# submarine0418/underwater_image_enhancement

Hardware: AMD Instinct MI355X
Metric: megapixels/sec enhanced (higher is better)
Workload: dtype f32/f64

## Files before the change

include/uwie.h:

```cpp
#ifndef UWIE_H_
#define UWIE_H_

#include <stddef.h>
#include <stdint.h>

#ifdef __cplusplus
extern "C" {
#endif

#define UWIE_OK 0
#define UWIE_E_INVALID (-1)
#define UWIE_E_WORKSPACE (-2)
#define UWIE_E_HIP (-3)
#define UWIE_E_NODEVICE (-4)
#define UWIE_E_DEVICE (-5)

#define UWIE_SURFACE_SIX 0
#define UWIE_SURFACE_DICT 1

#define UWIE_DICT_STRONG_DEHAZING 0
#define UWIE_DICT_MEDIUM_DEHAZING 1
#define UWIE_DICT_LIGHT_ENHANCEMENT 2
#define UWIE_DICT_CLAHE_ENHANCEMENT 3
#define UWIE_DICT_HISTOGRAM_EQUALIZATION 4
// ... 211 lines not shown
#define UWIE_MODEL_RF 0
#define UWIE_MODEL_GB 1
#define UWIE_MODEL_SVC 2
typedef struct uwie_model_desc {
    int32_t kind, n_features, n_classes, n_trees, n_nodes, n_sv;
    const double *mean, *scale;
    const int32_t *tree_offset, *left, *right, *feature;
    const double *threshold;
    const uint8_t *missing_left;
    const double *value;
    double learning_rate;
    const double *init;
    const double *sv, *dual_coef, *intercept;
    const int32_t *n_support;
    const double *prob_a, *prob_b;
    double gamma;
} uwie_model_desc;
typedef struct uwie_model uwie_model;

int uwie_model_check(const uwie_model_desc *desc);
int uwie_model_create(uwie_ctx *ctx, const uwie_model_desc *desc, uwie_model **out_model);
void uwie_model_destroy(uwie_model *model);
int uwie_model_info(const uwie_model *model, int *kind, int *n_classes, int *n_features);

int uwie_classify_f64(uwie_ctx *ctx, const uwie_model *model, const double *d_rows, int batch, int n_features, int32_t *d_label,
                      double *d_proba, void *stream);
size_t uwie_workspace_bytes_predict(int batch, int H, int W);
int uwie_predict_strategy_u8(uwie_ctx *ctx, const uwie_model *model, const uint8_t *d_u8, const float *d_f32, int batch, int H,
                             int W, int gray_shift, int32_t *d_label, double *d_proba, double *d_rows, void *d_workspace,
                             size_t workspace_bytes, void *stream);


int uwie_cast_classify(uwie_ctx *ctx, const uint8_t *d_in, int batch, int H, int W, int32_t *d_kind,
                       float *d_mean_rgb, void *d_workspace, size_t workspace_bytes, void *stream);

int uwie_normalise_correct(uwie_ctx *ctx, const uint8_t *d_in, const int32_t *d_kind, float *d_out_f32, int batch,
                           int H, int W, void *stream);

int uwie_atmospheric_light(uwie_ctx *ctx, const uint8_t *d_in, const int32_t *d_kind, int batch, int H, int W,
                           const uwie_params *p, float *d_A, void *d_trace, void *d_workspace,
                           size_t workspace_bytes, void *stream);

int uwie_transmission_init(uwie_ctx *ctx, const uint8_t *d_in, const int32_t *d_kind, const float *d_A, int batch,
                           int H, int W, const uwie_params *p, float *d_t0, uint8_t *d_gray, void *stream);

int uwie_box_filter_f64(uwie_ctx *ctx, const double *d_src, double *d_dst, int batch, int H, int W, int ksize,
                        void *d_workspace, size_t workspace_bytes, void *stream);

int uwie_guided_filter(uwie_ctx *ctx, const uint8_t *d_gray, const float *d_t0, int batch, int H, int W, int ksize,
                       double eps, int exact, double *d_t, void *d_workspace, size_t workspace_bytes, void *stream);

int uwie_guided_plan(int batch, int H, int W, int ksize, int *split_row0, int *split_rows);

int uwie_restore(uwie_ctx *ctx, const uint8_t *d_in, const int32_t *d_kind, const float *d_A, const double *d_t,
                 int batch, int H, int W, float *d_out_f32, void *stream);

int uwie_percentiles_f32(uwie_ctx *ctx, const float *d_img, int batch, int H, int W, const double *q_percent, int nq,
                         float *d_out, void *d_workspace, size_t workspace_bytes, void *stream);

int uwie_percentiles_f64(uwie_ctx *ctx, const double *d_img, int batch, int H, int W, const double *q_percent, int nq,
                         double *d_out, void *d_workspace, size_t workspace_bytes, void *stream);

int uwie_stretch_f32(uwie_ctx *ctx, const float *d_img, float *d_out, int batch, int H, int W, double lo_percent,
                     double hi_percent, void *d_workspace, size_t workspace_bytes, void *stream);

int uwie_gamma_f32(uwie_ctx *ctx, const float *d_img, float *d_out, size_t n, double g, int mode, void *stream);

int uwie_clahe_f32(uwie_ctx *ctx, const float *d_img, float *d_out, int batch, int H, int W, double clip_limit,
                   int tiles_x, int tiles_y, void *d_workspace, size_t workspace_bytes, void *stream);

int uwie_rgb2gray_u8(uwie_ctx *ctx, const uint8_t *d_rgb, uint8_t *d_gray, size_t npixels, int gray_shift,
                     void *stream);
int uwie_rgb2lab_u8(uwie_ctx *ctx, const uint8_t *d_rgb, uint8_t *d_lab, size_t npixels, void *stream);
int uwie_lab2rgb_u8(uwie_ctx *ctx, const uint8_t *d_lab, uint8_t *d_rgb, size_t npixels, void *stream);
int uwie_clahe_u8(uwie_ctx *ctx, const uint8_t *d_plane, uint8_t *d_out, int batch, int H, int W, double clip_limit,
                  int tiles_x, int tiles_y, void *d_workspace, size_t workspace_bytes, void *stream);
int uwie_canny_u8(uwie_ctx *ctx, const uint8_t *d_gray, uint8_t *d_edges, int batch, int H, int W, int low, int high,
                  void *d_workspace, size_t workspace_bytes, void *stream);
int uwie_equalize_hist_u8(uwie_ctx *ctx, const uint8_t *d_plane, uint8_t *d_out, int batch, int H, int W,
                          void *d_workspace, size_t workspace_bytes, void *stream);

#ifdef __cplusplus
}
#endif
#endif
```

profiles/gf_bench.py:

```python
import os
import sys
import time

import numpy as np
import torch

sys.path.insert(0, os.path.dirname(os.path.dirname(os.path.abspath(__file__))))
import underwater_image_enhancement_amd as uw

H, W, B = (int(v) for v in (sys.argv[1:4] if len(sys.argv) >= 4 else (2160, 3840, 16)))
k = int(sys.argv[4]) if len(sys.argv) > 4 else 15
eps = float(sys.argv[5]) if len(sys.argv) > 5 else 0.5
dev = uw.Device(0)
g = torch.Generator(device="cuda").manual_seed(1)
yy = torch.arange(H, device="cuda").view(1, H, 1)
xx = torch.arange(W, device="cuda").view(1, 1, W)
field = 0.5 + 0.25 * torch.sin(xx / 97.0) * torch.cos(yy / 61.0)
gray = (255 * (field + 0.03 * torch.randn((B, H, W), device="cuda", generator=g)).clamp(0, 1)).to(torch.uint8).contiguous()
t0 = (1.0 - 0.5 * (field * 0.9 + 0.05 * torch.rand((B, H, W), device="cuda", generator=g))).clamp(0.1, 1.0).float().contiguous()


def run(sel, exact=False, reps=5, kk=k):
    dev.tune(gf_split=1, gf_bands=0)
    dev.tune(**sel)
    t = dev.guided_filter(gray, t0, kk, eps, exact=exact)
    torch.cuda.synchronize()
    e0, e1 = torch.cuda.Event(enable_timing=True), torch.cuda.Event(enable_timing=True)
    e0.record()
    for _ in range(reps):
        t = dev.guided_filter(gray, t0, kk, eps, exact=exact)
    e1.record()
    torch.cuda.synchronize()
    return t, e0.elapsed_time(e1) / reps


nb = min(B, 2)
refs = {}
for kk in (k, 7):
    ref, ms_ref = run({}, exact=True, reps=1, kk=kk)
    refs[kk] = ref[:nb].clone()
    print(f"{H}x{W} x{B} k={kk} eps={eps}")
    print(f"  exact-order kernels      {ms_ref:8.3f} ms")
for name, env, mode, kk in (("LDS-tiled strip kernel", {}, False, 7), ("pipe, f64 ring in LDS", {"gf_split": 0}, False, k),
                            ("pipe, f64 split ring", {}, False, k), ("pipe, fx32 ring", {}, 2, k)):
    t, ms = run(env, exact=mode, kk=kk)
    err = (t[:nb] - refs[kk]).abs().max().item()
    gbs = B * H * W * 13 / ms / 1e6
    print(f"  {name:24s} k={kk:2d} {ms:8.3f} ms   {gbs:7.1f} GB/s algorithmic   max|t - t_exact| = {err:.3e}")
```

underwater_image_enhancement_amd/_lib.py:

```python
from __future__ import annotations

import ctypes
import os
import subprocess

_HERE = os.path.dirname(os.path.abspath(__file__))
LIB_PATH = os.path.join(_HERE, "lib", "libuwie.so")
CSRC = os.path.join(_HERE, "csrc")

SURFACE_SIX, SURFACE_DICT = 0, 1
STATUS_DIFF_RANK = 16
STATUS_CLASSIFY_NAN = 64
LOSS_IDENTITY, LOSS_VGG, LOSS_GATED = 0, 1, 2
VGG_F32, VGG_F16, VGG_PARAMS = 0, 1, 1735488
PARAM_NET_PARAMS = {True: 8500100, False: 8459652}
MASKS_GIVEN, MASKS_DRAWN = 0, 1
TRAINER_PARAMS, TRAINER_GRADS, TRAINER_EXP_AVG, TRAINER_EXP_AVG_SQ = 0, 1, 2, 3
FLIP_LR, FLIP_UD = 1, 2
RESIZE_MAX_SIDE, RESIZE_MAX_SRC = 4096, 32768
INTER_F64, INTER_FX32, INTER_F32T = 0, 1, 2
DICT_STRATEGIES = {
    "strong_dehazing": 0,
    "medium_dehazing": 1,
    "light_enhancement": 2,
# ... 21 lines not shown
        ("gf_eps", ctypes.c_double),
        ("L_low", ctypes.c_double),
        ("L_high", ctypes.c_double),
        ("wb_percentile", ctypes.c_double),
        ("clip_limit", ctypes.c_double),
        ("tiles_x", ctypes.c_int32),
        ("tiles_y", ctypes.c_int32),
        ("gamma", ctypes.c_double),
        ("apply_gamma", ctypes.c_int32),
        ("gf_exact", ctypes.c_int32),
        ("inter_dtype", ctypes.c_int32),
    ]


class UwieModelDesc(ctypes.Structure):

    _fields_ = [("kind", ctypes.c_int32), ("n_features", ctypes.c_int32), ("n_classes", ctypes.c_int32),
                ("n_trees", ctypes.c_int32), ("n_nodes", ctypes.c_int32), ("n_sv", ctypes.c_int32),
                ("mean", ctypes.c_void_p), ("scale", ctypes.c_void_p),
                ("tree_offset", ctypes.c_void_p), ("left", ctypes.c_void_p), ("right", ctypes.c_void_p),
                ("feature", ctypes.c_void_p), ("threshold", ctypes.c_void_p), ("missing_left", ctypes.c_void_p),
                ("value", ctypes.c_void_p), ("learning_rate", ctypes.c_double), ("init", ctypes.c_void_p),
                ("sv", ctypes.c_void_p), ("dual_coef", ctypes.c_void_p), ("intercept", ctypes.c_void_p),
                ("n_support", ctypes.c_void_p), ("prob_a", ctypes.c_void_p), ("prob_b", ctypes.c_void_p),
                ("gamma", ctypes.c_double)]


_VP, _SZ, _I, _D = ctypes.c_void_p, ctypes.c_size_t, ctypes.c_int, ctypes.c_double
_PP = ctypes.POINTER(UwieParams)
_PM = ctypes.POINTER(UwieModelDesc)
_PI = ctypes.POINTER(_I)
SIGNATURES = {
    "uwie_last_error": [],
    "uwie_version": [],
    "uwie_create": [_I, ctypes.POINTER(_VP)],
    "uwie_destroy": [_VP],
    "uwie_device_status": [_VP, _VP, ctypes.POINTER(ctypes.c_uint32)],
    "uwie_profile_enable": [_VP, _I],
    "uwie_profile_filter": [_VP, ctypes.c_char_p],
    "uwie_profile_collect": [_VP],
    "uwie_profile_row": [_VP, _I, ctypes.POINTER(ctypes.c_char_p), ctypes.POINTER(_D), ctypes.POINTER(_I)],
    "uwie_params_init": [_PP, _I, _I],
    "uwie_set_tuning": [_VP, ctypes.c_char_p, _I],
    "uwie_get_tuning": [_VP, ctypes.c_char_p, ctypes.POINTER(_I)],
    "uwie_workspace_bytes": [_I, _I, _I, _PP],
    "uwie_workspace_bytes_ctx": [_VP, _I, _I, _I, _PP],
    "uwie_workspace_bytes_all": [_I, _I, _I, _VP],
    "uwie_workspace_bytes_float": [_I, _I, _I, _PP, _I],
    "uwie_enhance_f32": [_VP, _VP, _VP, _VP, _VP, _I, _I, _I, _PP, _VP, _SZ, _VP],
    "uwie_enhance_f64": [_VP, _VP, _VP, _VP, _I, _I, _I, _PP, _VP, _SZ, _VP],
    "uwie_cast_classify_f32": [_VP, _VP, _I, _I, _I, _VP, _VP, _VP],
    "uwie_color_correct_f32": [_VP, _VP, _VP, _VP, _I, _I, _I, _VP],
    "uwie_guided_plan": [_I, _I, _I, _I, ctypes.POINTER(ctypes.c_int), ctypes.POINTER(ctypes.c_int)],
    "uwie_enhance_u8": [_VP, _VP, _VP, _VP, _I, _I, _I, _PP, _VP, _SZ, _VP],
    "uwie_enhance_u8_f64": [_VP, _VP, _VP, _VP, _I, _I, _I, _PP, _VP, _SZ, _VP],
    "uwie_enhance_percentiles": [_VP, _VP, _SZ, _I, _I, _I, _PP, _VP, _VP],
    "uwie_enhance_all_u8": [_VP, _VP, _VP, _VP, _I, _I, _I, _VP, _VP, _SZ, _VP],
    "uwie_workspace_bytes_select": [_I, _I, _I, _VP, _I, _I],
    "uwie_select_best_u8": [_VP, _VP, _I, _I, _I, _VP, _I, _VP, _VP, _VP, _VP, _VP, _VP, _SZ, _VP],
    "uwie_diff_enhance_f32": [_VP, _VP, _VP, _I, _I, _I, _I, _VP, _I, _VP, _SZ, _VP],
    "uwie_diff_enhance_save_f32": [_VP, _VP, _VP, _I, _I, _I, _I, _VP, _I, _VP, _VP, _SZ, _VP],
    "uwie_diff_enhance_bwd_workspace_bytes": [_I, _I, _I],
    "uwie_workspace_bytes_diff_u8": [_I, _I, _I],
    "uwie_diff_enhance_u8": [_VP, _VP, _VP, _VP, _I, _I, _I, _VP, _I, _VP, _VP, _SZ, _VP],
    "uwie_diff_enhance_bwd_f32": [_VP, _VP, _VP, _I, _I, _I, _I, _I, _VP, _VP, _VP, _VP, _VP, _SZ, _VP],
    "uwie_diff_gated_f32": [_VP, _VP, _VP, _I, _I, _I, _I, _VP, _I, _VP, _SZ, _VP],
    "uwie_diff_gated_save_f32": [_VP, _VP, _VP, _I, _I, _I, _I, _VP, _I, _VP, _VP, _SZ, _VP],
    "uwie_diff_gated_bwd_workspace_bytes": [_I, _I, _I],
    "uwie_workspace_bytes_diff_gated_u8": [_I],
    "uwie_diff_gated_u8": [_VP, _VP, _VP, _VP, _I, _I, _I, _VP, _I, _VP, _VP, _SZ, _VP],
    "uwie_diff_gated_bwd_f32": [_VP, _VP, _VP, _I, _I, _I, _I, _I, _VP, _VP, _VP, _VP, _VP, _SZ, _VP],
    "uwie_ref_loss_workspace_bytes": [_I, _I, _I],
    "uwie_ref_loss_f32": [_VP, _I, _VP, _VP, _I, _I, _I, _I, _I, _VP, _VP, _VP, _VP, _VP, _SZ, _VP],
    "uwie_ref_loss_bwd_f32": [_VP, _I, _VP, _VP, _I, _I, _I, _I, _I, _VP, _VP, _VP, _VP, _VP, _VP, _VP, _SZ, _VP],
    "uwie_device_status_async": [_VP, _VP, _VP],
    "uwie_vgg_create": [_VP, _VP, _I, ctypes.POINTER(_VP)],
    "uwie_vgg_destroy": [_VP],
    "uwie_perceptual_workspace_bytes": [_I, _I, _I, _I],
    "uwie_perceptual_f32": [_VP, _VP, _VP, _VP, _I, _I, _I, _VP, _VP, _SZ, _VP],
    "uwie_perceptual_bwd_f32": [_VP, _VP, _I, _I, _I, _VP, _VP, _VP, _SZ, _VP],
    "uwie_param_net_create": [_VP, _VP, _I, ctypes.POINTER(_VP)],
    "uwie_param_net_destroy": [_VP],
    "uwie_param_net_workspace_bytes": [_I, _I, _I],
    "uwie_param_net_f32": [_VP, _VP, _VP, _VP, _I, _I, _I, _VP, _VP, _VP, _SZ, _VP],
    "uwie_mlp_create": [_VP, _VP, _I, _I, _I, ctypes.POINTER(_VP)],
    "uwie_mlp_destroy": [_VP],
    "uwie_mlp_workspace_bytes": [_I, _I],
    "uwie_mlp_forward": [_VP, _VP, _VP, _I, _I, _VP, _VP, _SZ, _VP],
    "uwie_mlp_trainer_create": [_VP, _VP, _I, _I, _I, ctypes.POINTER(_VP)],
    "uwie_mlp_trainer_destroy": [_VP],
    "uwie_mlp_train_workspace_bytes": [_I, _I, _I],
    "uwie_mlp_train_forward": [_VP, _VP, _VP, _I, _I, _D, _I, _VP, ctypes.c_uint64, _VP, _VP, _SZ, _VP],
    "uwie_mlp_backward": [_VP, _VP, _VP, _I, _I, _VP, _VP, _SZ, _VP],
    "uwie_mlp_adam_step": [_VP, _VP, _D, _D, _D, _D, _D, _VP, _VP],
    "uwie_mlp_trainer_get": [_VP, _I, _VP],
    "uwie_mlp_trainer_set": [_VP, _I, _VP],
    "uwie_mlp_trainer_step_count": [_VP],
    "uwie_mlp_trainer_set_step_count": [_VP, ctypes.c_longlong],
    "uwie_mlp_trainer_eval": [_VP, _VP, _VP, _I, _I, _VP, _VP, _SZ, _VP],
    "uwie_u8_to_f32": [_VP, _VP, _VP, _SZ, _VP],
    "uwie_extract_features_u8": [_VP, _VP, _VP, _I, _I, _I, _VP, _SZ, _VP],
    "uwie_feature_extractor_count": [_I, _I],
    "uwie_workspace_bytes_feature_extractor": [_I, _I, _I],
    "uwie_feature_extractor_u8": [_VP, _VP, _VP, _I, _I, _I, _I, _VP, _VP, _SZ, _VP],
    "uwie_model_check": [_PM],
    "uwie_model_create": [_VP, _PM, ctypes.POINTER(_VP)],
# ... 85 lines not shown
```

underwater_image_enhancement_amd/csrc/api.hip:

```cpp
#include <cstdarg>
#include <cstdio>
#include <cstring>
#include <type_traits>

#include "common.h"

#include <cstdlib>

namespace uwie {

static thread_local char g_err[512] = "";
static thread_local uwie_ctx *g_ctx = nullptr;
static const Tuning g_default_tuning{};

const Tuning &tune() { return g_ctx ? g_ctx->tune : g_default_tuning; }
uwie_ctx *current_ctx() { return g_ctx; }

void set_error(const char *fmt, ...)
{
    va_list ap;
    va_start(ap, fmt);
    vsnprintf(g_err, sizeof g_err, fmt, ap);
    va_end(ap);
}
// ... 487 lines not shown
#define UWIE_REQUIRE_F(cond, ...)       \
    do {                                \
        if (!(cond)) {                  \
            set_error(__VA_ARGS__);     \
            return UWIE_E_INVALID;      \
        }                               \
    } while (0)

constexpr int kMlpEvalBatch = 1 << 20, kMlpTrainBatch = 65536;
template <class H>
int mlp_rows_check(const char *who, const uwie_ctx *ctx, const H *h, const void *d_features, int features_are_f64, int batch,
                   bool training, const float *d_other, const char *other_name)
{
    UWIE_REQUIRE_F(ctx && h && d_features && d_other, "%s: NULL pointer", who);
    UWIE_REQUIRE_F(h->device == ctx->device, "%s: the %s lives on another device", who,
                   std::is_same<H, uwie_mlp>::value ? "network" : "trainer");
    UWIE_REQUIRE_F(batch >= 1 && batch <= (training ? kMlpTrainBatch : kMlpEvalBatch), "%s: batch out of range (1 .. %s)", who,
                   training ? "65536" : "2^20");
    UWIE_REQUIRE_F(((uintptr_t)d_features & (features_are_f64 ? 7 : 3)) == 0 && ((uintptr_t)d_other & 3) == 0,
                   "%s: d_features and %s must be aligned for their element types", who, other_name);
    return UWIE_OK;
}

bool module_flags_ok(int map, int flags) { return map == UWIE_LOSS_VGG ? (flags & ~3) == 0 : flags == 0; }
int module_flags_check(const char *who, int map, int flags, bool name_module = false)
{
    const bool vgg = map == UWIE_LOSS_VGG;
    UWIE_REQUIRE_F(module_flags_ok(map, flags), "%s: %sflags are %s", who, !name_module ? "" : vgg ? "vgg " : "gated ",
                   vgg ? "UWIE_DIFF_OMEGA | UWIE_DIFF_GAMMA" : "reserved (0)");
    return UWIE_OK;
}

}
}

using namespace uwie;

extern "C" {

const char *uwie_last_error(void) { return g_err; }
const char *uwie_version(void) { return "uwie 0.1 (gfx950)"; }

int uwie_create(int device, uwie_ctx **out_ctx)
{
    UWIE_REQUIRE(out_ctx != nullptr, "out_ctx is NULL");
    *out_ctx = nullptr;
    int count = 0;
    if (hipGetDeviceCount(&count) != hipSuccess || count <= 0) {
        set_error("no HIP device available (libuwie has no CPU path)");
        return UWIE_E_NODEVICE;
    }
    UWIE_REQUIRE(device >= 0 && device < count, "device index out of range");
    UWIE_HIP_CHECK(hipSetDevice(device));
    uwie_ctx *ctx = new uwie_ctx();
    ctx->aux_ready = false;
    ctx->prof = prof_create();
    ctx->device = device;
    tuning_from_env(&ctx->tune);
    LabTables *lab = new LabTables();
    CastTables *cast = new CastTables();
    build_lab_tables(lab);
    build_cast_tables(cast);
    hipError_t e = hipMalloc((void **)&ctx->d_lab, sizeof(LabTables));
    if (e == hipSuccess) e = hipMalloc((void **)&ctx->d_cast, sizeof(CastTables));
    if (e == hipSuccess) e = hipMalloc((void **)&ctx->d_status, 64);
    if (e == hipSuccess) e = hipMemset(ctx->d_status, 0, 64);
    if (e == hipSuccess) e = hipMemcpy(ctx->d_lab, lab, sizeof(LabTables), hipMemcpyHostToDevice);
    if (e == hipSuccess) e = hipMemcpy(ctx->d_cast, cast, sizeof(CastTables), hipMemcpyHostToDevice);
    delete lab;
    delete cast;
    if (e != hipSuccess) {
        set_error("context table upload failed: %s", hipGetErrorString(e));
        uwie_destroy(ctx);
        return UWIE_E_HIP;
    }
    *out_ctx = ctx;
    return UWIE_OK;
}

void uwie_destroy(uwie_ctx *ctx)
{
    if (!ctx) return;
    if (ctx->d_lab) (void)hipFree(ctx->d_lab);
    if (ctx->d_cast) (void)hipFree(ctx->d_cast);
    if (ctx->d_status) (void)hipFree(ctx->d_status);
    if (ctx->aux_ready) {
        for (int i = 0; i < 4; ++i) {
            (void)hipStreamDestroy(ctx->aux[i]);
            (void)hipEventDestroy(ctx->join[i]);
        }
        (void)hipEventDestroy(ctx->fork);
    }
    prof_bind(nullptr);
    prof_destroy(ctx->prof);
    delete ctx;
}

int uwie_device_status(uwie_ctx *ctx, void *stream, uint32_t *bits)
{
    UWIE_REQUIRE(ctx != nullptr, "device_status: NULL context");
    UWIE_SCOPE(ctx);
    uint32_t v = 0;
    hipStream_t st = (hipStream_t)stream;
    UWIE_HIP_CHECK(hipMemcpyAsync(&v, ctx->d_status, sizeof v, hipMemcpyDeviceToHost, st));
    UWIE_HIP_CHECK(hipStreamSynchronize(st));
    if (v) UWIE_HIP_CHECK(hipMemsetAsync(ctx->d_status, 0, sizeof v, st));
    if (bits) *bits = v;
    if (v) {
        set_error("device status 0x%x:%s the results of the calls since the last check are not valid", v,
                  (v & UWIE_STATUS_CANNY_LABEL) ? " Canny hysteresis met a component label that this launch did not write (k_canny.hip);"
// ... 1202 lines not shown

int uwie_transmission_init(uwie_ctx *ctx, const uint8_t *d_in, const int32_t *d_kind, const float *d_A, int batch, int H,
                           int W, const uwie_params *p, float *d_t0, uint8_t *d_gray, void *stream)
{
    UWIE_REQUIRE(ctx && d_in && d_A && p && (d_t0 || d_gray), "transmission_init: NULL pointer");
    UWIE_SCOPE(ctx);
    UWIE_CHECK_SHAPE(batch, H, W);
    const Shape s{batch, H, W};
    hipStream_t st = (hipStream_t)stream;
    const bool six = p->surface == UWIE_SURFACE_SIX;
    if (d_t0) UWIE_TRY(launch_trans_init(d_in, d_kind, d_A, s, (float)p->omega, six ? 1e-6f : 1e-10f, six ? 1 : 0, d_t0, st));
    if (d_gray) UWIE_TRY(launch_quant_gray(d_in, d_kind, d_gray, s, p->gray_shift, st));
    return UWIE_OK;
}

int uwie_box_filter_f64(uwie_ctx *ctx, const double *d_src, double *d_dst, int batch, int H, int W, int ksize,
                        void *d_workspace, size_t workspace_bytes, void *stream)
{
    UWIE_REQUIRE(ctx && d_src && d_dst, "box_filter: NULL pointer");
    UWIE_SCOPE(ctx);
    UWIE_CHECK_SHAPE(batch, H, W);
    UWIE_REQUIRE(ksize >= 1 && ksize <= 1024, "box_filter: ksize out of range");
    const Shape s{batch, H, W};
    UWIE_CHECK_WS(box_ws_bytes(s));
    return launch_box_filter_f64(d_src, d_dst, s, ksize, d_workspace, (hipStream_t)stream);
}

int uwie_guided_filter(uwie_ctx *ctx, const uint8_t *d_gray, const float *d_t0, int batch, int H, int W, int ksize,
                       double eps, int exact, double *d_t, void *d_workspace, size_t workspace_bytes, void *stream)
{
    UWIE_REQUIRE(ctx && d_gray && d_t0 && d_t, "guided_filter: NULL pointer");
    UWIE_SCOPE(ctx);
    UWIE_CHECK_SHAPE(batch, H, W);
    UWIE_REQUIRE(ksize >= 1 && ksize <= 1024, "guided_filter: ksize out of range");
    const Shape s{batch, H, W};
    UWIE_CHECK_WS(guided_ws_bytes(s));
    UWIE_REQUIRE(exact >= 0 && exact <= 2, "guided_filter: mode is 0 (fused float64), 1 (exact order) or 2 (fixed-point ring)");
    GuidedRequest r{ksize, eps, exact == 1};
    r.fx = exact == 2;
    return launch_guided_plan(plan_guided(s, r), s, d_gray, d_t0, d_t, d_workspace, (hipStream_t)stream);
}

int uwie_guided_plan(int batch, int H, int W, int ksize, int *split_row0, int *split_rows)
{
    UWIE_REQUIRE(split_row0 && split_rows, "guided_plan: NULL pointer");
    UWIE_CHECK_SHAPE(batch, H, W);
    const GuidedPlan g = plan_guided(Shape{batch, H, W}, {ksize, 1.0});
    const bool split = g.route == GF_SPLIT;
    *split_row0 = split ? g.iy0 : 0;
    *split_rows = split ? g.rows : 0;
    return UWIE_OK;
}

int uwie_restore(uwie_ctx *ctx, const uint8_t *d_in, const int32_t *d_kind, const float *d_A, const double *d_t,
                 int batch, int H, int W, float *d_out_f32, void *stream)
{
    UWIE_REQUIRE(ctx && d_in && d_A && d_t && d_out_f32, "restore: NULL pointer");
    UWIE_SCOPE(ctx);
    UWIE_CHECK_SHAPE(batch, H, W);
    return launch_restore(d_in, d_kind, d_A, d_t, Shape{batch, H, W}, d_out_f32, (hipStream_t)stream);
}

int uwie_percentiles_f32(uwie_ctx *ctx, const float *d_img, int batch, int H, int W, const double *q_percent, int nq,
                         float *d_out, void *d_workspace, size_t workspace_bytes, void *stream)
{
    UWIE_REQUIRE(ctx && d_img && q_percent && d_out, "percentiles: NULL pointer");
    UWIE_SCOPE(ctx);
    UWIE_CHECK_SHAPE(batch, H, W);
    const Shape s{batch, H, W};
    UWIE_CHECK_WS(select_ws_bytes(s));
    return launch_percentiles(d_img, 0, s, q_percent, nq, d_out, d_workspace, (hipStream_t)stream);
}

int uwie_percentiles_f64(uwie_ctx *ctx, const double *d_img, int batch, int H, int W, const double *q_percent, int nq,
                         double *d_out, void *d_workspace, size_t workspace_bytes, void *stream)
{
    UWIE_REQUIRE(ctx && d_img && q_percent && d_out, "percentiles_f64: NULL pointer");
    UWIE_SCOPE(ctx);
    UWIE_CHECK_SHAPE(batch, H, W);
    const Shape s{batch, H, W};
    UWIE_CHECK_WS(select_ws_bytes(s));
    return launch_percentiles(d_img, 0, s, q_percent, nq, d_out, d_workspace, (hipStream_t)stream);
}

int uwie_enhance_percentiles(uwie_ctx *ctx, const void *d_workspace, size_t workspace_bytes, int batch, int H, int W,
                             const uwie_params *p, double *d_out, void *stream)
{
    UWIE_REQUIRE(ctx && d_workspace && d_out, "enhance_percentiles: NULL context, workspace or output pointer");
    UWIE_SCOPE(ctx);
    UWIE_CHECK_SHAPE(batch, H, W);
    UWIE_TRY(check_params(p));
    UWIE_REQUIRE(dehazes(p), "enhance_percentiles: only the dehazing strategies select percentiles in the workspace");
    const Shape s{batch, H, W};
    const EnhanceLayout L = carve_enhance(const_cast<void *>(d_workspace), workspace_bytes, s, p, !ctx->last_enhance_f64);
    UWIE_CHECK_WS(L.total);
    hipStream_t st = (hipStream_t)stream;
    const bool dict = p->surface == UWIE_SURFACE_DICT;
    const size_t per = (!dict && p->strategy == 3) ? 4 : 2;
    for (int i = 0; i < L.nsplit; ++i) {
        const size_t n = (size_t)L.cnt[i] * 3 * per;
        double *o = d_out + (size_t)L.start[i] * 3 * per;
        if (dict) UWIE_HIP_CHECK(hipMemcpyAsync(o, L.P[i].pct64, n * sizeof(double), hipMemcpyDeviceToDevice, st));
        else UWIE_TRY(launch_widen_f32(L.P[i].pct, o, n, st));
    }
    return UWIE_OK;
}
// ... 98 lines not shown
```

underwater_image_enhancement_amd/csrc/common.h:

```cpp
#pragma once
#include <hip/hip_runtime.h>
#include <stddef.h>
#include <stdint.h>

#include "../../include/uwie.h"

namespace uwie {

void set_error(const char *fmt, ...);
#define UWIE_HIP_CHECK(expr)                                                            \
    do {                                                                                \
        hipError_t _e = (expr);                                                         \
        if (_e != hipSuccess) {                                                         \
            ::uwie::set_error("%s failed: %s (%s:%d)", #expr, hipGetErrorString(_e), __FILE__, __LINE__); \
            return UWIE_E_HIP;                                                          \
        }                                                                               \
    } while (0)
#define UWIE_LAUNCH_CHECK() UWIE_HIP_CHECK(hipGetLastError())
#define UWIE_REQUIRE(cond, msg)                 \
    do {                                        \
        if (!(cond)) {                          \
            ::uwie::set_error("%s", msg);       \
            return UWIE_E_INVALID;              \
        }                                       \
// ... 16 lines not shown
    uint32_t R[kCastBinades][256];
    uint8_t tie[kCastBinades][256];
    uint32_t RT[256][kCastBinades];
    uint2 RT2[128][kCastBinades];
    uint8_t tiebin[256];
};

void build_lab_tables(LabTables *t);
void build_cast_tables(CastTables *t);

struct Profiler;
Profiler *prof_create();
void prof_destroy(Profiler *p);
void prof_enable(Profiler *p, bool on);
void prof_filter(Profiler *p, const char *name);
void prof_bind(Profiler *p);
int prof_collect(Profiler *p);
int prof_row(Profiler *p, int i, const char **name, double *ms, int *calls);
class ProfScope {
public:
    ProfScope(const char *name, hipStream_t st);
    ~ProfScope();
    ProfScope(const ProfScope &) = delete;

private:
    int rec_;
    hipStream_t st_;
};
#define UWIE_PROF_CAT2(a, b) a##b
#define UWIE_PROF_CAT(a, b) UWIE_PROF_CAT2(a, b)
#define UWIE_PROF(name, st) ::uwie::ProfScope UWIE_PROF_CAT(_uwie_prof_, __LINE__)(name, st)
#define UWIE_LAUNCH_AS(row, kernel, grid, block, lds, st, ...)              \
    do {                                                                    \
        UWIE_PROF(row, st);                                                 \
        hipLaunchKernelGGL(kernel, grid, block, lds, st, __VA_ARGS__);      \
    } while (0)
#define UWIE_LAUNCH(kernel, ...) UWIE_LAUNCH_AS(#kernel, kernel, __VA_ARGS__)

}

namespace uwie {
struct Tuning {
    int gf_split = 1;
    int gf_bands = 0;
    int select_generic = 0;
    int restore_store = 0;
    int lin_predict3 = 0;
    int lin_cap = 0;
    int lin_no_predict = 0;
    int q_hist = 1;
    int lin_predict_shift = 0;
    int streams = 1;
    int canny_prepass = 1;
    int gf_fuse = 0;
    int rank_sweep = 1;
    int canny_fault_inject = 0;
    int entry_fuse = 1;
};
const Tuning &tune();
uwie_ctx *current_ctx();
}

struct uwie_ctx {
    int device;
    uwie::Tuning tune;
    bool attr_q_tail = false;
    bool attr_cast_resolve = false;
    int attr_gf_fast = 0;
    int attr_gf_split8 = 0;
    uwie::LabTables *d_lab;
    uwie::CastTables *d_cast;
    uwie::Profiler *prof;
    uint32_t *d_status = nullptr;
    hipStream_t aux[4];
    hipEvent_t fork, join[4];
    bool aux_ready;
    bool last_enhance_f64 = false;
};

namespace uwie {

struct Carver {
    char *base;
    size_t off;
    explicit Carver(void *b) : base(static_cast<char *>(b)), off(0) {}
    template <typename T>
    T *take(size_t count)
    {
        off = (off + 255) & ~size_t(255);
        T *p = base ? reinterpret_cast<T *>(base + off) : nullptr;
        off += count * sizeof(T);
        return p;
    }
    size_t total() const { return (off + 255) & ~size_t(255); }
};

static inline int cdiv(long long a, long long b) { return (int)((a + b - 1) / b); }
static inline int grid_for(size_t n, size_t cap = 8192)
{
    size_t g = (n + 255) / 256;
    if (g > cap) g = cap;
    return g < 1 ? 1 : (int)g;
}

struct Region {
    int32_t img, y0, x0, rows, cols;
};

struct Shape {
    int B, H, W;
    size_t npx() const { return (size_t)H * W; }
};

size_t cast_ws_bytes(Shape s);
struct EntryFuse {
    uint32_t *qpart;
    uint8_t *gray;
    int32_t *guess;
    int gray_shift;
};
int launch_cast_classify(uwie_ctx *ctx, const uint8_t *d_in, Shape s, int32_t *d_kind, float *d_mean, void *ws,
                         hipStream_t st, const EntryFuse *ef = nullptr);
// ... 56 lines not shown
    const double *svT;
    const double *coef;
    const double *rho;
    const double *prob_a, *prob_b;
    const int32_t *sv_start;
};
int classify_model_check(const uwie_model_desc *d);
size_t classify_blob_bytes(const uwie_model_desc *d);
ClsModel classify_pack(const uwie_model_desc *d, void *host_blob, const void *dev_blob);
int launch_classify(const ClsModel &m, const double *d_rows, int B, int32_t *d_label, double *d_proba, uint32_t *d_status,
                    hipStream_t st);

int launch_pick_best(const double *d_scores, int n, Shape s, const uint8_t *d_all, int32_t *d_best, uint8_t *d_out, hipStream_t st);

size_t guided_ws_bytes(Shape s);
size_t box_ws_bytes(Shape s);
int launch_trans_init(const uint8_t *d_in, const int32_t *d_kind, const float *d_A, Shape s, float omega, float norm_eps,
                      int pre_clip, float *d_t0, hipStream_t st);
int launch_box_filter_f64(const double *d_src, double *d_dst, Shape s, int k, void *ws, hipStream_t st);
int launch_guided(const uint8_t *d_gray, const float *d_t0, Shape s, int k, double eps, double *d_t, void *ws,
                  hipStream_t st);
int launch_guided_p64(const uint8_t *d_gray, const double *d_t0, Shape s, int k, double eps, double *d_t, void *ws, hipStream_t st);

enum GuidedRoute {
    GF_EXACT,
    GF_FAST,
    GF_PIPE,
    GF_SPLIT,
    GF_FUSED,
};
struct GuidedRequest {
    int k;
    double eps;
    bool exact = false;
    bool fx = false;
    bool f32_ok = false;
    bool t0_from_frame = false;
    bool t0_f64 = false;
};
struct GuidedPlan {
    GuidedRoute route;
    int k;
    double eps;
    bool t_f32;
    bool ring_fx;
    bool t0_f64;
    bool t0;
    bool planes;
    int TH;
    int iy0, band, nb, rows;
    int pipe_bands;
};
GuidedPlan plan_guided(Shape s, const GuidedRequest &r);
struct FuseT0Args {
    const uint8_t *rgb;
    const int32_t *kind;
    const float *A;
    float omega, norm_eps;
    int pre_clip;
};
int launch_guided_plan(const GuidedPlan &g, Shape s, const uint8_t *d_gray, const void *d_t0, double *d_t, void *ws, hipStream_t st,
                       const FuseT0Args *frame = nullptr);
int guided_fast_th(Shape s, int k);
int launch_guided_fast(const uint8_t *d_gray, const float *d_t0, Shape s, int k, int TH, double eps, double *d_t, hipStream_t st);

constexpr int kMaxPct = 4;
size_t select_ws_bytes(Shape s);
template <typename V>
int launch_percentiles(const V *d_vals, int planar, Shape s, const double *q_percent, int nq, V *d_out, void *ws, hipStream_t st);
int launch_widen_f32(const float *d_in, double *d_out, size_t n, hipStream_t st);

constexpr int kSelGroupStride = 2 * kMaxPct * 2048;
constexpr int kSelOsStride = 2 * kMaxPct;
struct LinState;
struct SelectPlan {
    void *state;
    uint32_t *ghist;
    void *os;
    double t[kMaxPct];
    int nq;
    bool is64;
    LinState *lin;
    void *lists;
    uint32_t *flags;
    uint32_t cap;
    bool predicted;
    uint32_t ranks[2 * kMaxPct];
    template <typename V>
    V *lists_as() const { return static_cast<V *>(lists); }
};
constexpr int kLinBins = 2050;
__host__ __device__ inline uint32_t lin_digit(float x)
{
    if (!(x > 0.0f)) return 0;
    if (x >= 1.0f) return kLinBins - 1;
    const uint32_t d = (uint32_t)(x * 2048.0f);
    return 1 + (d > 2047u ? 2047u : d);
}
__host__ __device__ inline uint32_t lin_digit(double x)
{
    if (!(x > 0.0)) return 0;
    if (x >= 1.0) return kLinBins - 1;
    const uint32_t d = (uint32_t)(x * 2048.0);
    return 1 + (d > 2047u ? 2047u : d);
}
constexpr int kLinLists = 2 * kMaxPct;
// ... 164 lines not shown
```

underwater_image_enhancement_amd/csrc/k_guided_pipe.hip:

```cpp
#include "common.h"
#include "devutil.h"
#include "guided_wave.h"

#include <algorithm>
#include <cmath>
#include <type_traits>
#include <utility>

namespace uwie {

namespace {

#define UWIE_TRY_RC(call)               \
    do {                                \
        const int _rc = (call);         \
        if (_rc != UWIE_OK) return _rc; \
    } while (0)

#ifndef UWIE_GF_MINBAND
#define UWIE_GF_MINBAND 32
#endif
constexpr int kPipeSlots = 128;
struct PipeGeom {
    int H, W, band;
// ... 905 lines not shown
    int gr = i0 - Lb - 2;
    int yo = y_lo;
    auto issue = [&](In &fill) {
        asm volatile("" : "+s"(re), "+s"(gr), "+s"(yo));
        const uint32_t er = (uint32_t)pipe_reflect(re, H), lr = (uint32_t)pipe_reflect(re - RC, H);
        const uint32_t og = (uint32_t)min(max(gr, 0), H - 1);
        load_rows(er * pitch_t, er * pitch_g, lr * pitch_t, lr * pitch_g, og * pitch_g, fill);
        ++re;
        ++gr;
    };
    In buf[NB];
    [&]<int... Q>(std::integer_sequence<int, Q...>) { (issue(buf[Q]), ...); }(std::make_integer_sequence<int, NB - 1>{});
    auto one = [&](auto warm_tag, auto slot_tag, In &fill, const In &use) {
        issue(fill);
        step(warm_tag, slot_tag, use, (uint32_t)yo * pitch_o, yo < H);
        if constexpr (!decltype(warm_tag)::value) ++yo;
        __builtin_amdgcn_sched_barrier(0);
    };
    auto period = [&](auto warm_tag) {
        auto at = [&](auto slot_tag) {
            constexpr int S = decltype(slot_tag)::value;
            one(warm_tag, slot_tag, buf[(S + NB - 1) % NB], buf[S % NB]);
        };
        [&]<int... Q>(std::integer_sequence<int, Q...>) { (at(IC<Q>{}), ...); }(std::make_integer_sequence<int, RC>{});
    };
    period(std::true_type{});
    const int nper = (((int)bid.y == g.nbands - 1 ? g.y_end - y_lo : g.band) + RC - 1) / RC;
    for (int p = 0; p < nper; ++p) period(std::false_type{});
}


template <int K, typename TOut>
__global__ void __launch_bounds__(64) __attribute__((amdgpu_waves_per_eu(2, 2)))
k_guided_split(const uint8_t *__restrict__ gray, const float *__restrict__ t0, TOut *__restrict__ tout, SplitGeom g, PipeConsts cs)
{
    extern __shared__ double2 lds_raw[];
    char *lds = reinterpret_cast<char *>(lds_raw);
    int3 bid = {(int)blockIdx.x, (int)blockIdx.y, (int)blockIdx.z};
    if (g.xcd_fold) {
        const uint32_t gx = gridDim.x, gy = gridDim.y, n = gx * gy * gridDim.z;
        const uint32_t lin = blockIdx.x + gx * (blockIdx.y + gy * blockIdx.z);
        const uint32_t xcd = lin & 7u, idx = lin >> 3, q = n >> 3, r = n & 7u;
        const uint32_t log = (xcd < r ? xcd * (q + 1) : r * (q + 1) + (xcd - r) * q) + idx;
        bid.x = (int)(log % gx);
        bid.y = (int)((log / gx) % gy);
        bid.z = (int)(log / (gx * gy));
    }
    const int x_lo = bid.x * PipeCfg<K>::NV;
    const bool edge = x_lo - 2 * PipeCfg<K>::a < 0 || x_lo - 2 * PipeCfg<K>::a + kPipeSlots > g.W;
    if (edge) split_body<K, true, TOut>(gray, t0, tout, g, cs, lds, bid);
    else split_body<K, false, TOut>(gray, t0, tout, g, cs, lds, bid);
}

template <int K, typename TOut>
__global__ void __launch_bounds__(512) __attribute__((amdgpu_waves_per_eu(2, 2)))
k_guided_split8(const uint8_t *__restrict__ gray, FuseT0Args fz, TOut *__restrict__ tout, SplitGeom g, PipeConsts cs, int nstrips)
{
    extern __shared__ double2 lds_raw[];
    char *lds = reinterpret_cast<char *>(lds_raw);
    constexpr int per_wave = SplitCfg<K>::lds_bytes;
    float *tab = reinterpret_cast<float *>(lds + 8 * per_wave);
    const int wave = __builtin_amdgcn_readfirstlane((int)(threadIdx.x >> 6)), lane = threadIdx.x & 63;
    int grp = (int)blockIdx.x, b = (int)blockIdx.z;
    if (g.xcd_fold) {
        const uint32_t gx = gridDim.x, n = gx * gridDim.z, lin = blockIdx.x + gx * blockIdx.z;
        const uint32_t xcd = lin & 7u, idx = lin >> 3, q = n >> 3, r = n & 7u;
        const uint32_t log = (xcd < r ? xcd * (q + 1) : r * (q + 1) + (xcd - r) * q) + idx;
        grp = (int)(log % gx);
        b = (int)(log / gx);
    }
    {
        const int kd = fz.kind ? fz.kind[b] : 0;
        for (int i = threadIdx.x; i < 768; i += 512) {
            const int c = i >> 8;
            tab[i] = px_val(i & 255, px_atten(kd, c)) / (fz.A[b * 3 + c] + fz.norm_eps);
        }
    }
    __syncthreads();
    const int item = grp * 8 + wave;
    if (item >= nstrips * g.nbands) return;
    const int3 bid = {item % nstrips, item / nstrips, b};
    const int x_lo = bid.x * PipeCfg<K>::NV;
    const bool edge = x_lo - 2 * PipeCfg<K>::a < 0 || x_lo - 2 * PipeCfg<K>::a + kPipeSlots > g.W;
    const float *t0 = reinterpret_cast<const float *>(fz.rgb);
    if (edge) split_body<K, true, TOut, true>(gray, t0, tout, g, cs, lds + wave * per_wave, bid, lane, tab, fz.omega, fz.pre_clip);
    else split_body<K, false, TOut, true>(gray, t0, tout, g, cs, lds + wave * per_wave, bid, lane, tab, fz.omega, fz.pre_clip);
}

template <int K, typename TOut>
int launch_split8(const uint8_t *d_gray, const FuseT0Args &fz, Shape s, const PipeConsts &cs, TOut *d_t, int y0, int band, int nbands,
                  int y_end, hipStream_t st)
{
    using C = PipeCfg<K>;
    constexpr int lds = 8 * SplitCfg<K>::lds_bytes + 768 * 4;
    static_assert(lds <= 160 * 1024, "eight strips and the table have to fit one CU");
#ifndef UWIE_SPLIT8_FOLD
#define UWIE_SPLIT8_FOLD 1
#endif
    SplitGeom g{s.H, s.W, y0, band, y_end, UWIE_SPLIT8_FOLD, nbands};
    const int nstrips = cdiv(s.W, C::NV);
    uwie_ctx *ctx = current_ctx();
    const int bit = std::is_same<TOut, double>::value ? 1 : 2;
    if (ctx && !(ctx->attr_gf_split8 & bit)) {
        UWIE_HIP_CHECK(hipFuncSetAttribute(reinterpret_cast<const void *>(&k_guided_split8<K, TOut>),
                                           hipFuncAttributeMaxDynamicSharedMemorySize, lds));
        ctx->attr_gf_split8 |= bit;
    }
    {
        UWIE_PROF("k_guided_split8", st);
        hipLaunchKernelGGL((k_guided_split8<K, TOut>), dim3(cdiv((long long)nstrips * nbands, 8), 1, s.B), dim3(512), (size_t)lds, st, d_gray,
                           fz, d_t, g, cs, nstrips);
    }
    UWIE_LAUNCH_CHECK();
    return UWIE_OK;
}

template <int K, typename TOut>
int launch_split(const uint8_t *d_gray, const float *d_t0, Shape s, const PipeConsts &cs, TOut *d_t, int y0, int band, int nbands,
                 int y_end, hipStream_t st)
{
    using C = PipeCfg<K>;
    constexpr int lds = SplitCfg<K>::lds_bytes;
#ifndef UWIE_SPLIT_FOLD
#define UWIE_SPLIT_FOLD 1
#endif
    SplitGeom g{s.H, s.W, y0, band, y_end, UWIE_SPLIT_FOLD, nbands};
    const int nstrips = cdiv(s.W, C::NV);
    {
        UWIE_PROF("k_guided_split", st);
        hipLaunchKernelGGL((k_guided_split<K, TOut>), dim3(nstrips, nbands, s.B), dim3(64), (size_t)lds, st, d_gray, d_t0, d_t, g, cs);
    }
    UWIE_LAUNCH_CHECK();
    return UWIE_OK;
}

template <int K, bool FX, typename TOut>
int launch_pipe(const uint8_t *d_gray, const float *d_t0, Shape s, const PipeConsts &cs, TOut *d_t, int nbands, hipStream_t st,
                const int *border = nullptr)
{
    using C = PipeCfg<K>;
    constexpr int lds = C::lds_bytes(FX);
    const int nstrips = cdiv(s.W, C::NV);
    PipeGeom g{};
    g.H = s.H; g.W = s.W;
    g.band = cdiv(s.H, nbands);
    int gy = cdiv(s.H, g.band);
    if (border) {
        g.iy0 = border[0]; g.iy1 = border[1]; g.iband = border[2];
        gy = 2 + border[3];
        g.is0 = border[4]; g.is1 = border[5];
    }
    {
        UWIE_PROF("k_guided_pipe", st);
        hipLaunchKernelGGL((k_guided_pipe<K, FX, TOut>), dim3(nstrips, gy, s.B), dim3(64), (size_t)lds, st, d_gray, d_t0, d_t, g, cs);
    }
    UWIE_LAUNCH_CHECK();
    return UWIE_OK;
}

int pipe_bands(Shape s, int k, bool fx, int forced)
{
    const int lds = k == 10 ? PipeCfg<10>::lds_bytes(fx) : k == 15 ? PipeCfg<15>::lds_bytes(fx) : PipeCfg<20>::lds_bytes(fx);
    const int resident = 256 * std::max(1, std::min(8, (160 * 1024) / lds));
// ... 45 lines not shown
    const double amax = (se <= 0.5 ? 0.45 / (2.0 * se) : 0.225 / (0.25 + eps)) * 1.02;
    const double hb = (0.45 + amax) * 1.02;
    *Sa = (int)std::floor(std::log2(1073741824.0 / amax));
    *Sb = (int)std::floor(std::log2(1073741824.0 / hb));
    return *Sa >= 28 && *Sb >= 28;
}

PipeConsts pipe_consts(const GuidedPlan &g)
{
    const double K2 = (double)g.k * g.k, scale = 1.0 / K2;
    PipeConsts cs{};
    cs.Ek = 255.0 * K2 * K2 * g.eps;
    cs.kaI = scale / 255.0;
    cs.kb = scale;
    cs.b0 = 0.0;
    int Sa, Sb;
    if (g.ring_fx && fx_scales(g.eps, &Sa, &Sb)) {
        const double fa = std::ldexp(1.0, Sa), fb = std::ldexp(1.0, Sb);
        const double b0i = std::nearbyint(0.55 * fb);
        cs.fxa = fa;
        cs.fxb = scale * fb;
        cs.magic_b = kMagic - b0i;
        cs.kaI = scale / 255.0 / fa;
        cs.kb = scale / fb;
        cs.b0 = b0i / fb;
    }
    return cs;
}

template <int K, typename TOut>
int launch_pipe_plan(const GuidedPlan &g, const uint8_t *d_gray, const float *d_t0, Shape s, const PipeConsts &cs, TOut *d_t,
                     hipStream_t st)
{
    if constexpr (std::is_same<TOut, double>::value)
        if (g.ring_fx) return launch_pipe<K, true, double>(d_gray, d_t0, s, cs, d_t, g.pipe_bands, st);
    if (g.route == GF_PIPE) return launch_pipe<K, false, TOut>(d_gray, d_t0, s, cs, d_t, g.pipe_bands, st);
    UWIE_TRY_RC((launch_split<K, TOut>(d_gray, d_t0, s, cs, d_t, g.iy0, g.band, g.nb, g.iy0 + g.rows, st)));
    if (K & 1) return UWIE_OK;
    const int border[6] = {g.iy0, g.iy0 + g.rows, g.band, 0, 0, 0};
    return launch_pipe<K, false, TOut>(d_gray, d_t0, s, cs, d_t, g.pipe_bands, st, border);
}

template <typename TOut>
int launch_wave(const GuidedPlan &g, const uint8_t *d_gray, const float *d_t0, Shape s, TOut *d_t, hipStream_t st)
{
    const PipeConsts cs = pipe_consts(g);
    if (g.k == 10) return launch_pipe_plan<10>(g, d_gray, d_t0, s, cs, d_t, st);
    if (g.k == 15) return launch_pipe_plan<15>(g, d_gray, d_t0, s, cs, d_t, st);
    return launch_pipe_plan<20>(g, d_gray, d_t0, s, cs, d_t, st);
}

}

GuidedPlan plan_guided(Shape s, const GuidedRequest &r)
{
    GuidedPlan g{};
    g.k = r.k;
    g.eps = r.eps;
    g.t0 = true;
    const bool free_order = !r.exact && !r.t0_f64 && r.k >= 1 && r.k <= 1024;
    const bool wave = free_order && (r.k == 10 || r.k == 15 || r.k == 20) && s.W >= 2 * r.k && s.H >= 4 * r.k && s.B <= 65535 &&
                      r.eps > 0.0;
    if (!wave) {
        g.TH = free_order ? guided_fast_th(s, r.k) : 0;
        g.route = g.TH ? GF_FAST : GF_EXACT;
        g.t0_f64 = r.t0_f64;
        g.planes = !g.TH;
        return g;
    }
    const Tuning &tu = tune();
    int Sa, Sb;
    g.ring_fx = r.fx && fx_scales(r.eps, &Sa, &Sb);
    g.t_f32 = r.f32_ok && !g.ring_fx && !(s.W & 1);
    g.pipe_bands = pipe_bands(s, r.k, g.ring_fx, tu.gf_bands);
    g.route = GF_PIPE;
    if (!g.ring_fx && tu.gf_split && split_plan(s, r.k, tu.gf_bands, &g.iy0, &g.band, &g.nb, &g.rows)) {
        g.route = GF_SPLIT;
        if (r.k == 15 && r.t0_from_frame && !r.fx && tu.gf_fuse) {
            g.route = GF_FUSED;
            g.t0 = false;
        }
    }
    return g;
}

int launch_guided_plan(const GuidedPlan &g, Shape s, const uint8_t *d_gray, const void *d_t0, double *d_t, void *ws, hipStream_t st,
                       const FuseT0Args *frame)
{
    const float *t0 = static_cast<const float *>(d_t0);
    switch (g.route) {
    case GF_EXACT:
        UWIE_REQUIRE(ws, "guided filter: the exact-order kernels need the workspace's planes");
        if (g.t0_f64) return launch_guided_p64(d_gray, static_cast<const double *>(d_t0), s, g.k, g.eps, d_t, ws, st);
        return launch_guided(d_gray, t0, s, g.k, g.eps, d_t, ws, st);
    case GF_FAST: return launch_guided_fast(d_gray, t0, s, g.k, g.TH, g.eps, d_t, st);
    case GF_FUSED:
        UWIE_REQUIRE(frame, "guided filter: the fused plan computes t0 from the frame");
        if (g.t_f32) return launch_split8<15, float>(d_gray, *frame, s, pipe_consts(g), reinterpret_cast<float *>(d_t), g.iy0, g.band, g.nb, s.H, st);
        return launch_split8<15, double>(d_gray, *frame, s, pipe_consts(g), d_t, g.iy0, g.band, g.nb, s.H, st);
    default:
        if (g.t_f32) return launch_wave(g, d_gray, t0, s, reinterpret_cast<float *>(d_t), st);
        return launch_wave(g, d_gray, t0, s, d_t, st);
    }
}

}
```

Baseline: 57860.

## Enable fused t0 guided-filter route by default when strips fill the GPU

Changes the default gf_fuse from 0 to 2. In mode 2 the fused split8 kernel, which computes t0 from the frame inside the guided filter, is chosen only when the number of strip work items covers at least one full round of resident wavefronts (8 per compute unit). The split8 kernel also drops from 8 to 4 waves per block, so two blocks can share a CU and tail blocks can be smaller. A query API and a sweep benchmark are added to compare the fused and unfused routes. The aim is to skip the separate t0 pass and its memory traffic on large batches, while keeping the unfused path for small batches where the fused kernel would leave the GPU underfilled.

```diff
diff --git a/include/uwie.h b/include/uwie.h
--- a/include/uwie.h
+++ b/include/uwie.h
@@ -287,6 +287,8 @@
 
 int uwie_guided_plan(int batch, int H, int W, int ksize, int *split_row0, int *split_rows);
 
+int uwie_guided_fill(int batch, int H, int W, int ksize, long long *items);
+
 int uwie_restore(uwie_ctx *ctx, const uint8_t *d_in, const int32_t *d_kind, const float *d_A, const double *d_t,
                  int batch, int H, int W, float *d_out_f32, void *stream);
 
diff --git a/profiles/gf_bench.py b/profiles/gf_bench.py
--- a/profiles/gf_bench.py
+++ b/profiles/gf_bench.py
@@ -7,6 +7,57 @@
 
 sys.path.insert(0, os.path.dirname(os.path.dirname(os.path.abspath(__file__))))
 import underwater_image_enhancement_amd as uw
+
+
+
+def sweep():
+    import ctypes
+
+    from underwater_image_enhancement_amd import _lib
+
+    REPS = 5
+    dev = uw.Device(0)
+    cus = torch.cuda.get_device_properties(0).multi_processor_count
+    p = dev.params(_lib.SURFACE_SIX, 2)
+    print(f"# gf_fuse = 1 against 0, strategy 2, ms per call (min .. max of three alternating rounds of {REPS} calls); {cus} compute units,")
+    print(f"# resident strip-wavefronts {cus * 8}; default: the route gf_fuse = 2 takes")
+    print("# H W B items rounds | fuse=0 ms | fuse=1 ms | median diff ms | default route")
+    jobs = [(2160, 3840, b) for b in (2, 4, 8, 16, 32, 64)] + [(1080, 1920, b) for b in (10, 64, 128)]
+    for H, W, B in jobs:
+        g = torch.Generator(device="cuda").manual_seed(B)
+        frames = torch.randint(0, 256, (B, H, W, 3), generator=g, device="cuda", dtype=torch.uint8)
+        items = ctypes.c_longlong()
+        _lib.check(dev.lib.uwie_guided_fill(B, H, W, 15, ctypes.byref(items)))
+        ms = {0: [], 1: []}
+        for rnd in range(4):
+            for fuse in (0, 1):
+                with dev.tuning(gf_fuse=fuse):
+                    dev.enhance_u8(frames, p)
+                    e0, e1 = torch.cuda.Event(enable_timing=True), torch.cuda.Event(enable_timing=True)
+                    e0.record()
+                    for _ in range(REPS):
+                        dev.enhance_u8(frames, p)
+                    e1.record()
+                    torch.cuda.synchronize()
+                if rnd:
+                    ms[fuse].append(e0.elapsed_time(e1) / REPS)
+        dev.profile(True)
+        dev.profile_rows()
+        dev.enhance_u8(frames, p)
+        rows = dev.profile_rows()
+        dev.profile(False)
+        route = "fused" if "k_guided_split8" in rows else "split" if "k_guided_split" in rows else "pipe"
+        med = sorted(ms[1])[1] - sorted(ms[0])[1]
+        print(f"{H} {W} {B:3d} {items.value:6d} {items.value / (cus * 8):5.2f} | {min(ms[0]):7.3f} .. {max(ms[0]):7.3f} | "
+              f"{min(ms[1]):7.3f} .. {max(ms[1]):7.3f} | {med:+7.3f} | {route}", flush=True)
+        del frames
+        dev._workspace = None
+        torch.cuda.empty_cache()
+
+
+if len(sys.argv) > 1 and sys.argv[1] == "--sweep":
+    sweep()
+    sys.exit(0)
 
 H, W, B = (int(v) for v in (sys.argv[1:4] if len(sys.argv) >= 4 else (2160, 3840, 16)))
 k = int(sys.argv[4]) if len(sys.argv) > 4 else 15
diff --git a/underwater_image_enhancement_amd/_lib.py b/underwater_image_enhancement_amd/_lib.py
--- a/underwater_image_enhancement_amd/_lib.py
+++ b/underwater_image_enhancement_amd/_lib.py
@@ -97,6 +97,7 @@
     "uwie_cast_classify_f32": [_VP, _VP, _I, _I, _I, _VP, _VP, _VP],
     "uwie_color_correct_f32": [_VP, _VP, _VP, _VP, _I, _I, _I, _VP],
     "uwie_guided_plan": [_I, _I, _I, _I, ctypes.POINTER(ctypes.c_int), ctypes.POINTER(ctypes.c_int)],
+    "uwie_guided_fill": [_I, _I, _I, _I, ctypes.POINTER(ctypes.c_longlong)],
     "uwie_enhance_u8": [_VP, _VP, _VP, _VP, _I, _I, _I, _PP, _VP, _SZ, _VP],
     "uwie_enhance_u8_f64": [_VP, _VP, _VP, _VP, _I, _I, _I, _PP, _VP, _SZ, _VP],
     "uwie_enhance_percentiles": [_VP, _VP, _SZ, _I, _I, _I, _PP, _VP, _VP],
diff --git a/underwater_image_enhancement_amd/csrc/api.hip b/underwater_image_enhancement_amd/csrc/api.hip
--- a/underwater_image_enhancement_amd/csrc/api.hip
+++ b/underwater_image_enhancement_amd/csrc/api.hip
@@ -563,10 +563,13 @@
     }
     UWIE_REQUIRE(device >= 0 && device < count, "device index out of range");
     UWIE_HIP_CHECK(hipSetDevice(device));
+    int cus = 0;
+    UWIE_HIP_CHECK(hipDeviceGetAttribute(&cus, hipDeviceAttributeMultiprocessorCount, device));
     uwie_ctx *ctx = new uwie_ctx();
     ctx->aux_ready = false;
     ctx->prof = prof_create();
     ctx->device = device;
+    ctx->cus = cus;
     tuning_from_env(&ctx->tune);
     LabTables *lab = new LabTables();
     CastTables *cast = new CastTables();
@@ -1875,6 +1878,16 @@
     return UWIE_OK;
 }
 
+int uwie_guided_fill(int batch, int H, int W, int ksize, long long *items)
+{
+    UWIE_REQUIRE(items, "guided_fill: NULL pointer");
+    UWIE_CHECK_SHAPE(batch, H, W);
+    const Shape s{batch, H, W};
+    const GuidedPlan g = plan_guided(s, {ksize, 1.0});
+    *items = g.route == GF_SPLIT ? guided_items(s, g) : 0;
+    return UWIE_OK;
+}
+
 int uwie_restore(uwie_ctx *ctx, const uint8_t *d_in, const int32_t *d_kind, const float *d_A, const double *d_t,
                  int batch, int H, int W, float *d_out_f32, void *stream)
 {
diff --git a/underwater_image_enhancement_amd/csrc/common.h b/underwater_image_enhancement_amd/csrc/common.h
--- a/underwater_image_enhancement_amd/csrc/common.h
+++ b/underwater_image_enhancement_amd/csrc/common.h
@@ -92,7 +92,7 @@
     int lin_predict_shift = 0;
     int streams = 1;
     int canny_prepass = 1;
-    int gf_fuse = 0;
+    int gf_fuse = 2;
     int rank_sweep = 1;
     int canny_fault_inject = 0;
     int entry_fuse = 1;
@@ -108,6 +108,7 @@
     bool attr_cast_resolve = false;
     int attr_gf_fast = 0;
     int attr_gf_split8 = 0;
+    int cus = 0;
     uwie::LabTables *d_lab;
     uwie::CastTables *d_cast;
     uwie::Profiler *prof;
@@ -270,6 +271,7 @@
     int pipe_bands;
 };
 GuidedPlan plan_guided(Shape s, const GuidedRequest &r);
+inline long long guided_items(Shape s, const GuidedPlan &g) { return (long long)cdiv(s.W, 128 - 2 * (g.k - 1)) * g.nb * s.B; }
 struct FuseT0Args {
     const uint8_t *rgb;
     const int32_t *kind;
diff --git a/underwater_image_enhancement_amd/csrc/k_guided_pipe.hip b/underwater_image_enhancement_amd/csrc/k_guided_pipe.hip
--- a/underwater_image_enhancement_amd/csrc/k_guided_pipe.hip
+++ b/underwater_image_enhancement_amd/csrc/k_guided_pipe.hip
@@ -981,14 +981,18 @@
     else split_body<K, false, TOut>(gray, t0, tout, g, cs, lds, bid);
 }
 
+#ifndef SPLIT8_WAVES
+#define SPLIT8_WAVES 4
+#endif
 template <int K, typename TOut>
-__global__ void __launch_bounds__(512) __attribute__((amdgpu_waves_per_eu(2, 2)))
+__global__ void __launch_bounds__(64 * SPLIT8_WAVES) __attribute__((amdgpu_waves_per_eu(2, 2)))
 k_guided_split8(const uint8_t *__restrict__ gray, FuseT0Args fz, TOut *__restrict__ tout, SplitGeom g, PipeConsts cs, int nstrips)
 {
     extern __shared__ double2 lds_raw[];
     char *lds = reinterpret_cast<char *>(lds_raw);
     constexpr int per_wave = SplitCfg<K>::lds_bytes;
-    float *tab = reinterpret_cast<float *>(lds + 8 * per_wave);
+    constexpr int NW = SPLIT8_WAVES;
+    float *tab = reinterpret_cast<float *>(lds + NW * per_wave);
     const int wave = __builtin_amdgcn_readfirstlane((int)(threadIdx.x >> 6)), lane = threadIdx.x & 63;
     int grp = (int)blockIdx.x, b = (int)blockIdx.z;
     if (g.xcd_fold) {
@@ -1000,13 +1004,13 @@
     }
     {
         const int kd = fz.kind ? fz.kind[b] : 0;
-        for (int i = threadIdx.x; i < 768; i += 512) {
+        for (int i = threadIdx.x; i < 768; i += 64 * NW) {
             const int c = i >> 8;
             tab[i] = px_val(i & 255, px_atten(kd, c)) / (fz.A[b * 3 + c] + fz.norm_eps);
         }
     }
     __syncthreads();
-    const int item = grp * 8 + wave;
+    const int item = grp * NW + wave;
     if (item >= nstrips * g.nbands) return;
     const int3 bid = {item % nstrips, item / nstrips, b};
     const int x_lo = bid.x * PipeCfg<K>::NV;
@@ -1021,8 +1025,9 @@
                   int y_end, hipStream_t st)
 {
     using C = PipeCfg<K>;
-    constexpr int lds = 8 * SplitCfg<K>::lds_bytes + 768 * 4;
-    static_assert(lds <= 160 * 1024, "eight strips and the table have to fit one CU");
+    constexpr int NW = SPLIT8_WAVES;
+    constexpr int lds = NW * SplitCfg<K>::lds_bytes + 768 * 4;
+    static_assert(8 % NW == 0 && (8 / NW) * lds <= 160 * 1024, "eight strips and their tables have to fit one CU");
 #ifndef UWIE_SPLIT8_FOLD
 #define UWIE_SPLIT8_FOLD 1
 #endif
@@ -1037,7 +1042,7 @@
     }
     {
         UWIE_PROF("k_guided_split8", st);
-        hipLaunchKernelGGL((k_guided_split8<K, TOut>), dim3(cdiv((long long)nstrips * nbands, 8), 1, s.B), dim3(512), (size_t)lds, st, d_gray,
+        hipLaunchKernelGGL((k_guided_split8<K, TOut>), dim3(cdiv((long long)nstrips * nbands, NW), 1, s.B), dim3(64 * NW), (size_t)lds, st, d_gray,
                            fz, d_t, g, cs, nstrips);
     }
     UWIE_LAUNCH_CHECK();
@@ -1189,6 +1194,8 @@
 
 }
 
+constexpr long long kFuseRounds = 1;
+
 GuidedPlan plan_guided(Shape s, const GuidedRequest &r)
 {
     GuidedPlan g{};
@@ -1214,8 +1221,12 @@
     if (!g.ring_fx && tu.gf_split && split_plan(s, r.k, tu.gf_bands, &g.iy0, &g.band, &g.nb, &g.rows)) {
         g.route = GF_SPLIT;
         if (r.k == 15 && r.t0_from_frame && !r.fx && tu.gf_fuse) {
-            g.route = GF_FUSED;
-            g.t0 = false;
+            const uwie_ctx *ctx = current_ctx();
+            const long long resident = 8LL * (ctx ? ctx->cus : 0);
+            if (tu.gf_fuse == 1 || (tu.gf_fuse == 2 && resident > 0 && guided_items(s, g) >= kFuseRounds * resident)) {
+                g.route = GF_FUSED;
+                g.t0 = false;
+            }
         }
     }
     return g;
```

After: 60050, median of 6. 3.8% higher.
